# Yzmblog/SurfD

Measured on AMD Instinct MI355X. Metric: shapes/sec end-to-end (1000-step uncond, 512^3 UDF) at 1/2/4/8 GPU, higher is better.
Workload: dtype f32 (every matrix product of decoder and denoiser as three split-fp16 products on the fp16 MFMA pipe with fp32 accumulation — fp32-class error, same golden tolerances as the exact-fp32 kernels; samplers, attention, embedding MLP and grid bookkeeping in exact fp32)

## Files before the change

surfd_amd/csrc/conv_f16x2.hip:

```cpp
#include "common.h"
#include "unet_api.h"
#include "unet_plan.h"
#include <string.h>
#include <stdlib.h>
#include <algorithm>
#include <type_traits>

namespace surfd {

typedef _Float16 f16x8 __attribute__((ext_vector_type(8)));
typedef f16x8 __attribute__((address_space(1))) gf16x8;
typedef _Float16 f16x2 __attribute__((ext_vector_type(2)));
typedef float f32x2 __attribute__((ext_vector_type(2)));

struct Seg2 {
    const float *x;
    long bstride;
    const float *gamma, *beta;
    int C, Lin, log2Lin;
    int taps, stride, ups, gn, act;
    int blk, blkp, nblk;
    int k16_off;
    int gs;
    int log2P, gsm;
};

struct Conv2Args {
    Seg2 seg[2];
    int nseg;
    const _Float16 *whf;
    int KS16;
#if defined(SURFD_C2_PROBE) || defined(SURFD_C2_DBG_POISON)
    unsigned long long *probe;
#define C2_LDS_BYTES plane
#else
    const float *sc;
#endif
    float inv_sc;
    const float *bias;
    const float *emb;
    long emb_bstride;
    const float *res;
    long res_bstride;
    int res_cstride, res_lstride, has_res, has_emb;
    float *out;
    long out_bstride;
    int Cout, Lout, log2Lout, B;
    int bchunk, Lsl, cs;
    int plane;
    int off_ex, off_red;
    int ntiles, nby, KS;
    int nrt;
    int nhalf;
    unsigned magic_nby, magic_ks, magic_g;
    float *part;
    int part_stride;
    int *counters;
    const int *step_ptr;
    long emb_step_stride;
// ... 263 lines not shown
        "s_mov_b32 s66, %0\n\ts_mov_b32 s67, %0\n\ts_mov_b32 s68, %0\n\ts_mov_b32 s69, %0\n\ts_mov_b32 s70, %0\n\ts_mov_b32 s71, %0\n\t"
        "s_mov_b32 s72, %0\n\ts_mov_b32 s73, %0\n\ts_mov_b32 s74, %0\n\ts_mov_b32 s75, %0\n\ts_mov_b32 s76, %0\n\ts_mov_b32 s77, %0\n\t"
        "s_mov_b32 s78, %0\n\ts_mov_b32 s79, %0\n\ts_mov_b32 s80, %0\n\ts_mov_b32 s81, %0\n\ts_mov_b32 s82, %0\n\ts_mov_b32 s83, %0\n\t"
        "s_mov_b32 s84, %0\n\ts_mov_b32 s85, %0\n\ts_mov_b32 s86, %0\n\ts_mov_b32 s87, %0\n\ts_mov_b32 s88, %0\n\ts_mov_b32 s89, %0\n\t"
        "s_mov_b32 s90, %0\n\ts_mov_b32 s91, %0\n\ts_mov_b32 s92, %0\n\ts_mov_b32 s93, %0\n\ts_mov_b32 s94, %0\n\ts_mov_b32 s95, %0\n\t"
        "s_mov_b32 s96, %0\n\ts_mov_b32 s97, %0\n\ts_mov_b32 s98, %0\n\ts_mov_b32 s99, %0\n\t"
        "s_nop 0"
        :: "s"(pat)
        :
          "v1","v2","v3","v4","v5","v6","v7","v8","v9","v10","v11","v12","v13","v14","v15","v16","v17","v18","v19","v20","v21","v22","v23","v24",
          "v25","v26","v27","v28","v29","v30","v31","v32","v33","v34","v35","v36","v37","v38","v39","v40","v41","v42","v43","v44","v45","v46","v47","v48",
          "v49","v50","v51","v52","v53","v54","v55","v56","v57","v58","v59","v60","v61","v62","v63","v64","v65","v66","v67","v68","v69","v70","v71","v72",
          "v73","v74","v75","v76","v77","v78","v79","v80","v81","v82","v83","v84","v85","v86","v87","v88","v89","v90","v91","v92","v93","v94","v95","v96",
          "v97","v98","v99","v100","v101","v102","v103","v104","v105","v106","v107","v108","v109","v110","v111","v112","v113","v114","v115","v116","v117","v118","v119","v120",
          "v121","v122","v123","v124","v125","v126","v127","v128","v129","v130","v131","v132","v133","v134","v135","v136","v137","v138","v139","v140","v141","v142","v143","v144",
          "v145","v146","v147","v148","v149","v150","v151","v152","v153","v154","v155","v156","v157","v158","v159",
          "s4","s5","s6","s7","s8","s9","s10","s11","s12","s13","s14","s15","s16","s17","s18","s19","s20","s21","s22","s23","s24","s25","s26","s27",
          "s28","s29","s30","s31","s34","s35","s36","s37","s38","s39","s40","s41","s42","s43","s44","s45","s46","s47","s48","s49","s50","s51","s52","s53",
          "s54","s55","s56","s57","s58","s59","s60","s61","s62","s63","s64","s65","s66","s67","s68","s69","s70","s71","s72","s73","s74","s75","s76","s77",
          "s78","s79","s80","s81","s82","s83","s84","s85","s86","s87","s88","s89","s90","s91","s92","s93","s94","s95","s96","s97","s98","s99");
}
#endif

template <int VEC, bool PREF, bool WT = false, bool LEAN = false, bool LF = false, bool NT2 = false>
__global__ __launch_bounds__(256, LEAN ? SURFD_C2_LEAN_WAVES : (VEC == 16 ? (WT ? 2 : 1) : 2)) void conv2_kernel(Conv2Args A) {
    static_assert(!LEAN || (WT && VEC == 8 && !PREF), "lean form: wide decomposition, rows of <= 32 positions, no operand prefetch");
    static_assert(!NT2 || (LEAN && !LF), "two column tiles per wave: lean form only");
    constexpr int NCT = NT2 ? 2 : 1;
    [[maybe_unused]] constexpr int EXS = NT2 ? 128 : 256;
    constexpr bool SLIM = LEAN || (WT && VEC == 16);
    constexpr bool ONE_ACC = NT2 || (LEAN && SURFD_C2_LEAN_U == 3);
    constexpr int C2_U = (LEAN && !NT2) ? SURFD_C2_LEAN_U : SLIM ? 2 : 4;
    constexpr int C2_D = (VEC == 8 && SURFD_C2_EPI_LATE && !LEAN && !LF) ? (WT ? SURFD_C2_DEEP_D : SURFD_C2_LAT_D) : 2;
    [[maybe_unused]] constexpr bool ALIAS = SLIM;
    extern __shared__ __attribute__((aligned(16))) char lds_raw[];
    _Float16 *slab = reinterpret_cast<_Float16 *>(lds_raw);
#if !SURFD_C2_GNW
    float *ex_mean = reinterpret_cast<float *>(lds_raw + (ALIAS ? 0 : A.off_ex));
    float *ex_m2 = ex_mean + VEC * 256;
    float *gstat = ex_m2 + VEC * 256;
#endif
    float *red = reinterpret_cast<float *>(lds_raw + A.off_red);

#if defined(SURFD_C2_DBG_POISON) && SURFD_C2_DBG_POISON
    c2_poison_registers<!LEAN>();
    for (int e = threadIdx.x; e < A.C2_LDS_BYTES / 4; e += 256) reinterpret_cast<unsigned *>(lds_raw)[e] = SURFD_C2_DBG_POISON == 2 ? 0x7fc00000u : 0u;
    lds_bar();
#endif
    c2_kernarg_prefetch<(int)sizeof(Conv2Args)>();
    const int tid = threadIdx.x, lane = tid & 63;
    const int wave = __builtin_amdgcn_readfirstlane(tid >> 6);
#ifdef SURFD_C2_STAMPS
    long long stamp_[12];
#pragma unroll
    for (int i = 0; i < 12; ++i) stamp_[i] = 0;
#define C2_STAMP(i) do { stamp_[i] = (long long)__builtin_amdgcn_s_memrealtime(); } while (0)
#define C2_STAMP_FIRST(i) do { if (ch == kz) C2_STAMP(i); } while (0)
#else
#define C2_STAMP(i) do { } while (0)
#define C2_STAMP_FIRST(i) do { } while (0)
#endif
    C2_STAMP(0);
#ifdef SURFD_C2_STAMPS
    const long long cyc0_ = (long long)__builtin_readcyclecounter();
#endif
    int tile, by, kz, rg;
    bool tile_ok = true;
    {
        const int bid = blockIdx.x;
        const int G = A.nrt * A.KS;
        int g;
        if (G < 8) {
            by = G == 1 ? bid : (int)__umulhi((unsigned)bid, A.magic_g);
            g = bid - by * G;
        } else {
            const int xcd = bid & 7, idx = bid >> 3;
            const int j = A.nby == 1 ? idx : (int)__umulhi((unsigned)idx, A.magic_nby);
            by = idx - j * A.nby;
            g = xcd + 8 * j;
            if (g >= G) return;
        }
        rg = A.KS == 1 ? g : (int)__umulhi((unsigned)g, A.magic_ks);
        kz = g - rg * A.KS;
        tile = rg;
        if constexpr (WT) {
            tile = rg * 4 + wave;
            tile_ok = tile < A.ntiles;
            tile = min(tile, A.ntiles - 1);
        }
    }
    const bool halves = WT && A.nhalf == 2;
// ... 14 lines not shown
        const int lp = A.seg[s].log2P, gsm = A.seg[s].gsm;
        const int pos = lane & ((1 << lp) - 1);
        const int c = ((wc << (6 - lp)) + (lane >> lp)) * gsm + pos;
        ok = pos < gsm && c < A.seg[s].blk;
        return c;
#else
        ok = zthr < A.seg[s].blk;
        return zthr;
#endif
    };
    int colb[NCT], coll[NCT];
#pragma unroll
    for (int t = 0; t < NCT; ++t) {
        int m = (NT2 ? t : ct) * 32 + (lane & 31);
        if (m >= M) m = 0;
        m += m_off;
        colb[t] = m >> A.log2Lout;
        coll[t] = m & (A.Lout - 1);
    }
    const int nblk0 = A.seg[0].nblk;
    const int nch = nblk0 + (A.nseg > 1 ? A.seg[1].nblk : 0);
    constexpr int PLANE = NT2 ? C2_PLANE_NT2 : LEAN ? C2_PLANE_LEAN : (VEC == 16 ? 18432 : 15360);
    const int cs = A.cs;
    const float inv_sc = A.inv_sc;

    f32x16 acc_hh[NCT], acc_sm[1];
#pragma unroll
    for (int t = 0; t < NCT; ++t)
#pragma unroll
        for (int r = 0; r < 16; ++r) acc_hh[t][r] = 0.f;
    if constexpr (!ONE_ACC)
#pragma unroll
        for (int r = 0; r < 16; ++r) acc_sm[0][r] = 0.f;

    struct WS { const _Float16 *base; int it_beg, it_end, ngroups, nk; };
    auto make_ws = [&](int ch) -> WS {
        const int s = ch >= nblk0 ? 1 : 0;
        const int bi = ch - (s ? nblk0 : 0);
        const int nk = A.seg[s].blkp >> 4;
        const int iters = A.seg[s].taps * nk;
        const int per = (iters + KP - 1) >> log2kp;
        WS w;
        w.nk = nk;
        w.it_beg = min(kpart * per, iters);
        w.it_end = min(iters, w.it_beg + per);
        w.ngroups = (per + C2_U - 1) / C2_U;
// ... 17 lines not shown

    auto issue_operand = [&](int ch, f32x4 (&v)[VEC], float &ga, float &be) {
        const int s = ch >= nblk0 ? 1 : 0;
        const int bi = ch - (s ? nblk0 : 0);
        const int lv = A.seg[s].log2Lin - 2;
        const int Lin = A.seg[s].Lin;
        bool cok_;
        const int cg = min(bi * A.seg[s].blk + min(chan_of(s, cok_), A.seg[s].blk - 1), A.seg[s].C - 1);
        const float *src = A.seg[s].x + (long)cg * Lin;
        const long bstride = A.seg[s].bstride;
        const int rowbase = rhalf * ((VEC * 4) >> A.seg[s].log2Lin);
#pragma unroll
        for (int j = 0; j < VEC; ++j) {
            const int i = min(rowbase + (j >> lv), nb - 1), jj = j & ((1 << lv) - 1);
            v[j] = *reinterpret_cast<const f32x4 *>(src + (b0 + i) * bstride + 4 * jj);
        }
        ga = A.seg[s].gamma[cg]; be = A.seg[s].beta[cg];
    };

    int ch = kz;
    WS cur = make_ws(ch);
    f32x4 v[VEC];
    float ga, be;
    issue_operand(ch, v, ga, be);
#pragma unroll
    for (int d = 0; d < C2_D; ++d) load_group(ring[d], cur.base, cur.it_beg + d * C2_U, cur.it_end - 1);
    unsigned pf_sink[C2_PFN_N];
    if constexpr (SURFD_C2_PFN_FORMS || LEAN) c2_prefetch_next(A, tid, pf_sink);
    else {
#pragma unroll
        for (int k = 0; k < C2_PFN_N; ++k) pf_sink[k] = 0u;
    }

    f32x4 pre_b[4], pre_e[NCT][4];
    float pre_r[NCT][16];
    const float *embp = A.emb;
    if (A.step_ptr) embp += (long)(*reinterpret_cast<const __attribute__((address_space(4))) int *>((unsigned long)A.step_ptr)) * A.emb_step_stride;
    LoopFuse lfv;
    int lfk = 0;
    float lfrow[5] = {0.f, 0.f, 0.f, 0.f, 0.f};
    if constexpr (LF) {
        lfv = *A.lf;
        lfk = *lfv.step;
#pragma unroll
        for (int q = 0; q < 5; ++q) lfrow[q] = lfv.tab[(long)lfk * 8 + q];
    }
    auto request_epilogue = [&]() {
        const int cmax4 = ((A.Cout + 3) & ~3) - 4;
#pragma unroll
        for (int t = 0; t < NCT; ++t) {
            const int m = min((NT2 ? t : ct) * 32 + (lane & 31), M - 1) + m_off;
// ... 26 lines not shown
#pragma unroll
        for (int qq = 0; qq < 2; ++qq) {
            const int q = kpart * QN + min(qq, QN - 1);
            const int cob = min(tile * 32 + 8 * q + 4 * (lane >> 5), cmax4);
            dpre_b[qq] = *reinterpret_cast<const f32x4 *>(A.bias + cob);
            dpre_e[qq] = *reinterpret_cast<const f32x4 *>(embp + b * A.emb_bstride + cob);
#pragma unroll
            for (int k = 0; k < 4; ++k) {
                const int co = min(cob + k, A.Cout - 1);
                dpre_r[qq][k] = A.res[b * A.res_bstride + (long)co * A.res_cstride + l * A.res_lstride];
            }
        }
    };
    constexpr bool EPI_LATE = SLIM || SURFD_C2_EPI_LATE;
    if constexpr (!EPI_LATE && !DIST) request_epilogue();
    bool saturated = false;
    C2_STAMP(1);
#ifdef SURFD_C2_PROBE
    unsigned long long probe_w = 0ull;
#endif

    while (true) {
        {
            const int s = ch >= nblk0 ? 1 : 0;
            const int bi = ch - (s ? nblk0 : 0);
            const int lv = A.seg[s].log2Lin - 2, vpr = 1 << lv;
            const int Lin = A.seg[s].Lin;
            const int blk = A.seg[s].blk, blkp = A.seg[s].blkp;
            bool cok;
            const int c = chan_of(s, cok);
            const int rowbase = rhalf * ((VEC * 4) >> A.seg[s].log2Lin);
            const int pad = A.seg[s].taps == 3 ? 1 : 0;
            const int ups = A.seg[s].ups, act = A.seg[s].act;
#ifdef SURFD_C2_PROBE
            {
                unsigned long long h = 0ull;
#pragma unroll
                for (int j = 0; j < VEC; ++j)
#pragma unroll
                    for (int k = 0; k < 4; ++k) h += (unsigned long long)__float_as_uint(v[j][k]) * (unsigned long long)(2 * ((ch * 256 + tid) * 64 + j * 4 + k) + 1);
                h += (unsigned long long)__float_as_uint(ga) * 7ull + (unsigned long long)__float_as_uint(be) * 11ull;
                C2_PROBE_ADD(0, h);
            }
#endif
            if (A.seg[s].gn) {
                const int gs = A.seg[s].gs;
// ... 187 lines not shown
                                const f32x2 hf = __builtin_convertvector(h, f32x2);
                                const f16x2 lo = __builtin_convertvector(w - hf, f16x2);
                                _Float16 *d0 = row + (k * RS) * cs, *d1 = d0 + RS * cs;
                                d0[0] = h[0]; d0[PLANE] = lo[0];
                                d1[0] = h[1]; d1[PLANE] = lo[1];
                                if constexpr (UPS) { d0[cs] = h[0]; d0[cs + PLANE] = lo[0]; d1[cs] = h[1]; d1[cs + PLANE] = lo[1]; }
                            }
                        }
                    }
                };
                if (ups) split_rows(std::true_type{}); else split_rows(std::false_type{});
                saturated |= amax > 65504.f;
            }
            if (zthr >= blk && zthr < blkp) {
                for (int i = 0; i < nb; ++i)
                    for (int p = 0; p < A.Lsl; ++p) { slab[(i * A.Lsl + p) * cs + zthr] = (_Float16)0.f; slab[(i * A.Lsl + p) * cs + zthr + PLANE] = (_Float16)0.f; }
            }
            if (cok)
                for (int i = 0; i < nb; ++i) {
                    _Float16 *row0 = slab + (i * A.Lsl) * cs + c;
                    for (int p = 0; p < pad; ++p) { row0[p * cs] = (_Float16)0.f; row0[p * cs + PLANE] = (_Float16)0.f; }
                    for (int p = pad + Lcov; p < A.Lsl; ++p) { row0[p * cs] = (_Float16)0.f; row0[p * cs + PLANE] = (_Float16)0.f; }
                }
            lds_bar();
            C2_STAMP_FIRST(4);
#ifdef SURFD_C2_PROBE
            {
                unsigned long long h = 0ull;
                const int n = nb * A.Lsl * blkp;
                for (int e = tid; e < n; e += 256) {
                    const int cch = e % blkp, rp = e / blkp;
                    const unsigned short hi = __builtin_bit_cast(unsigned short, slab[rp * cs + cch]), lo = __builtin_bit_cast(unsigned short, slab[rp * cs + cch + PLANE]);
                    h += ((unsigned long long)hi + 65537ull * lo) * (unsigned long long)(2 * (ch * 65536 + e) + 1);
                }
                C2_PROBE_ADD(3, h);
                lds_bar();
            }
#endif
        }
        const int chn = ch + A.KS;
        const bool has_next = chn < nch;
        const WS nxt = has_next ? make_ws(chn) : cur;
        f32x4 vn[PREF ? VEC : 1];
        float gan = 0.f, ben = 0.f;
        if constexpr (PREF) issue_operand(has_next ? chn : ch, vn, gan, ben);
        {
            const int s = ch >= nblk0 ? 1 : 0;
            int lbase[NCT];
#pragma unroll
            for (int t = 0; t < NCT; ++t) lbase[t] = (colb[t] * A.Lsl + coll[t] * A.seg[s].stride) * cs + 8 * (lane >> 5);
// ... 72 lines not shown
#pragma unroll
                for (int d = 0; d < C2_D; ++d) {
                    const int g = g0 + d;
                    compute(ring[d], g);
                    const int vg = g + C2_D;
                    const bool into_next = has_next && vg >= P;
                    const _Float16 *rb = into_next ? nxt.base : cur.base;
                    const int it0 = into_next ? nxt.it_beg + (vg - P) * C2_U : cur.it_beg + vg * C2_U;
                    const int itl = into_next ? nxt.it_end - 1 : cur.it_end - 1;
                    load_group(ring[d], rb, it0, itl);
                }
                g0 += C2_D;
            } while (g0 < P);
        }
        C2_STAMP_FIRST(5);
        if (!has_next) break;
        lds_bar();
        ch = chn;
        cur = nxt;
        if constexpr (PREF) {
#pragma unroll
            for (int j = 0; j < VEC; ++j) v[j] = vn[j];
            ga = gan; be = ben;
        } else {
            issue_operand(ch, v, ga, be);
        }
    }
    if constexpr (DIST) request_epilogue_dist();
    else if constexpr (EPI_LATE) request_epilogue();
    if (saturated) atomicAdd(A.sat, 1u);
    C2_STAMP(6);

    if constexpr (DIST) {
        lds_bar();
        {
            float *dst = red + (kpart * nct + ct) * 1024;
#pragma unroll
            for (int r = 0; r < 16; ++r) dst[r * 64 + lane] = ONE_ACC ? acc_hh[0][r] : acc_sm[0][r] + acc_hh[0][r];
        }
        lds_bar();
        f32x4 val[2];
#pragma unroll
        for (int qq = 0; qq < 2; ++qq) {
            const int q = kpart * QN + min(qq, QN - 1);
            const float *srcp = red + ct * 1024 + (4 * q) * 64 + lane;
            f32x4 t = {srcp[0], srcp[64], srcp[128], srcp[192]};
            for (int kp = 1; kp < KP; ++kp) {
// ... 199 lines not shown
            const int prev = __hip_atomic_fetch_add(lfv.done, 1, __ATOMIC_RELAXED, __HIP_MEMORY_SCOPE_AGENT);
            if (prev == A.nby * A.nrt - 1) {
                __hip_atomic_store(lfv.done, 0, __ATOMIC_RELAXED, __HIP_MEMORY_SCOPE_AGENT);
                __hip_atomic_store(lfv.step, lfk + 1, __ATOMIC_RELAXED, __HIP_MEMORY_SCOPE_AGENT);
            }
        }
    }
    {
        unsigned used = 0u;
#pragma unroll
        for (int k = 0; k < C2_PFN_N; ++k) used |= pf_sink[k];
        asm volatile("" :: "v"(used));
    }
#ifdef SURFD_C2_STAMPS
    C2_STAMP(9);
    asm volatile("s_waitcnt vmcnt(0)" ::: "memory");
    C2_STAMP(10);
    if (A.dbg && blockIdx.x == 0 && tid == 0) {
        for (int i = 0; i < 11; ++i) A.dbg[i] = stamp_[i];
        A.dbg[15] = (long long)__builtin_readcyclecounter() - cyc0_;
    }
#endif
}

__global__ void c2_hash_kernel(const float *p, long bstride, int B, int row, unsigned long long *out) {
    unsigned long long h = 0ull;
    const long n = (long)B * row;
    for (long e = blockIdx.x * (long)blockDim.x + threadIdx.x; e < n; e += (long)gridDim.x * blockDim.x) {
        const long b = e / row, r = e - b * row;
        h += (unsigned long long)__float_as_uint(p[b * bstride + r]) * (unsigned long long)(2 * e + 1);
    }
#pragma unroll
    for (int off = 32; off > 0; off >>= 1) h += __shfl_xor(h, off);
    if ((threadIdx.x & 63) == 0) atomicAdd(out, h);
}

__global__ void c2_absmax_kernel(const float *src, size_t n, unsigned *out) {
    unsigned m = 0u;
    for (size_t i = blockIdx.x * (size_t)blockDim.x + threadIdx.x; i < n; i += (size_t)gridDim.x * blockDim.x)
        m = max(m, __float_as_uint(src[i]) & 0x7fffffffu);
#pragma unroll
    for (int off = 32; off > 0; off >>= 1) m = max(m, (unsigned)__shfl_xor((int)m, off));
    if ((threadIdx.x & 63) == 0 && m) atomicMax(out, m);
}

__global__ void c2_scale_kernel(float *sc) {
// ... 303 lines not shown
    } else {
        if (base < ks_min_base && nch > 1) KS = std::min({nch, ks_max, std::max(1, ks_fill / base)});
        if ((size_t)KS * base * A.part_stride > u->part_floats || base > 8192) KS = 1;
    }
    A.KS = KS;
    static const int deep_below = env_int("SURFD_CONV2_DEEP_BELOW", 0);
    if (lean && !nt2 && deep_below > 0 && (long)A.nrt * KS * A.nby <= (long)deep_below * u->cu_budget) {
        lean = false;
        lds = (size_t)15360 * 2 * sizeof(_Float16);
        lds = (lds + 15) & ~(size_t)15;
        A.plane = 15360; A.off_ex = (int)lds; A.off_red = (int)lds;
#if SURFD_C2_GNW
        lds += (size_t)(4 * 1024 + 4) * sizeof(float);
#else
        lds += std::max(((size_t)2 * VEC * 256 + 2 * 8 * 32) * sizeof(float), (size_t)(3 * 1024 + 4) * sizeof(float));
#endif
        lds += (size_t)lds_extra;
        lds = (lds + 255) & ~(size_t)255;
        A.off_pf = (int)lds;
        lds += 256;
    }
    A.part = u->part; A.counters = u->counters;
    A.sat = u->sat;
    if (fuse_head) {
        if (io.ext_out_bs != (long)c.Cout * A.Lout) SURFD_FAIL(SURFD_ERR_ARG, "conv: fused posterior update needs a contiguous head output");
        A.lf = io.lf;
        if (io.lf_done) *io.lf_done = true;
    }
    A.dbg = nullptr;
    if (u->dbg && u->dbg_launch < 4096) {
        A.dbg = u->dbg + (size_t)(u->dbg_launch++) * 16;
        long long meta[4] = {c.Cout, c.seg[0].C + (c.nseg > 1 ? c.seg[1].C : 0), A.Lout * 100000LL + (long long)A.ntiles * A.nby * KS, KS * 100 + nch};
        HIP_TRY(hipMemcpyAsync(A.dbg + 11, meta, sizeof(meta), hipMemcpyHostToDevice, st));
    }
    A.magic_nby = (unsigned)((0x100000000ULL + A.nby - 1) / A.nby);
    A.magic_ks = (unsigned)((0x100000000ULL + KS - 1) / KS);
    const int G = A.nrt * KS;
    A.magic_g = (unsigned)((0x100000000ULL + G - 1) / G);
    if ((long)G * A.nby >= 65536) SURFD_FAIL(SURFD_ERR_UNSUPPORTED, "conv: %d x %d workgroups exceed the kernel's block decode", G, A.nby);
    dim3 grid((unsigned)(G < 8 ? G * A.nby : 8 * ceil_div(G, 8) * A.nby));
    static const int pref = env_int("SURFD_CONV2_PREF", 0);
    static const int wpref = env_int("SURFD_CONV2_WIDE_PREF", 0);
    {
        ConvPlan::LaunchRec &R = c.rec;
        R.gen = u->ws_gen; R.B = B; R.L = L; R.whf = A.whf; R.ntiles = A.ntiles; R.KS16 = A.KS16; R.tpg = wt ? 4 : 1; R.KS = KS; R.G = A.nrt * KS;
        R.nblk0 = A.seg[0].nblk; R.it0 = A.seg[0].taps * (A.seg[0].blkp >> 4);
// ... 11 lines not shown
            A.pf_w = reinterpret_cast<const char *>(R.whf);
            A.pf_ntiles = R.ntiles; A.pf_KS16 = R.KS16; A.pf_KS = R.KS; A.pf_G = R.G;
            A.pf_nblk0 = R.nblk0; A.pf_it0 = R.it0; A.pf_nch = R.nch; A.pf_it1 = std::max(R.it1, 1);
            auto lg = [](int v) { int l = 0; while ((1 << l) < v) ++l; return l; };
            A.pf_log2tpg = lg(R.tpg); A.pf_log2bps = lg(ceil_div(R.nch, R.KS)); A.pf_log2lpb = lg(16 * std::max(R.it0, R.it1));
            A.pf_magic_ks = (unsigned)((0x100000000ULL + R.KS - 1) / R.KS);
        }
    }
#if defined(SURFD_C2_PROBE) || defined(SURFD_C2_DBG_POISON)
    {
        static unsigned long long *const probe_base = [] { const char *e = getenv("SURFD_CONV2_PROBE_PTR"); return e ? reinterpret_cast<unsigned long long *>(strtoull(e, nullptr, 0)) : nullptr; }();
        A.probe = (probe_base && grid.x <= 4096 && c.id < 128) ? probe_base + (size_t)c.id * 4096 * 8 : nullptr;
        A.C2_LDS_BYTES = (int)lds;
    }
#endif
    auto launch = [&]() {
        if (A.lf) {
            if (wt && VEC == 16) hipLaunchKernelGGL((conv2_kernel<16, false, true, false, true>), grid, dim3(256), lds, st, A);
            else if (wt) hipLaunchKernelGGL((conv2_kernel<8, false, true, false, true>), grid, dim3(256), lds, st, A);
            else if (VEC == 16) hipLaunchKernelGGL((conv2_kernel<16, false, false, false, true>), grid, dim3(256), lds, st, A);
            else hipLaunchKernelGGL((conv2_kernel<8, false, false, false, true>), grid, dim3(256), lds, st, A);
        }
        else if (nt2) hipLaunchKernelGGL((conv2_kernel<8, false, true, true, false, true>), grid, dim3(256), lds, st, A);
        else if (lean) hipLaunchKernelGGL((conv2_kernel<8, false, true, true>), grid, dim3(256), lds, st, A);
        else if (wt && VEC == 16) hipLaunchKernelGGL((conv2_kernel<16, false, true>), grid, dim3(256), lds, st, A);
        else if (wt && wpref) hipLaunchKernelGGL((conv2_kernel<8, true, true>), grid, dim3(256), lds, st, A);
        else if (wt) hipLaunchKernelGGL((conv2_kernel<8, false, true>), grid, dim3(256), lds, st, A);
        else if (VEC == 16) hipLaunchKernelGGL((conv2_kernel<16, false>), grid, dim3(256), lds, st, A);
        else if (pref) hipLaunchKernelGGL((conv2_kernel<8, true>), grid, dim3(256), lds, st, A);
        else hipLaunchKernelGGL((conv2_kernel<8, false>), grid, dim3(256), lds, st, A);
    };
    launch();
    LAUNCH_CHECK();
    static const int hash_env = env_int("SURFD_CONV2_HASH", 0);
    if (hash_env && A.dbg) {
        HIP_TRY(hipMemsetAsync(A.dbg, 0, sizeof(long long), st));
        hipLaunchKernelGGL(c2_hash_kernel, dim3(64), dim3(256), 0, st, (const float *)A.out, (long)A.out_bstride, B, A.Cout * A.Lout,
                           reinterpret_cast<unsigned long long *>(A.dbg));
        LAUNCH_CHECK();
    }
    static const int twice = env_int("SURFD_CONV2_TWICE", 0);
    if (twice && !A.lf) {
        if (A.dbg && u->dbg_launch < 4096) {
            long long *prev = A.dbg;
            A.dbg = u->dbg + (size_t)(u->dbg_launch++) * 16;
            HIP_TRY(hipMemcpyAsync(A.dbg + 11, prev + 11, 4 * sizeof(long long), hipMemcpyDeviceToDevice, st));
        }
        launch();
    }
    LAUNCH_CHECK();
    return SURFD_OK;
}

#define C2_STR_(x) #x
// ... 28 lines not shown
#error "SURFD_C2_GNPAD=0: the in-wave GroupNorm reductions without wait states are NOT bit-stable run to run (profiles/r05_loop_experiments.md section 3, profiles/r06_conv2_instability.md); -DSURFD_ALLOW_UNSAFE_VARIANTS builds it anyway"
#endif
#if SURFD_C2_LAT_D != 2
#error "SURFD_C2_LAT_D != 2 is not a validated configuration of the latency form (profiles/r05_loop_experiments.md section 1); -DSURFD_ALLOW_UNSAFE_VARIANTS builds it anyway"
#endif
#if SURFD_C2_BPIPE == 2
#error "SURFD_C2_BPIPE=2 is the control of an experiment (not bit-stable with SURFD_C2_GNW, profiles/r06_conv2_instability.md); -DSURFD_ALLOW_UNSAFE_VARIANTS builds it anyway"
#endif
#if C2_CFG_ABLATE != 0 || C2_CFG_POISON != 0 || C2_CFG_PROBE != 0
#error "developer aids of conv_f16x2.hip (SURFD_C2_ABLATE / _DBG_POISON / _PROBE) change results or timing; -DSURFD_ALLOW_UNSAFE_VARIANTS builds them anyway"
#endif
#endif
const char *conv2_build_config() {
    return "C2_GNW=" C2_STR(SURFD_C2_GNW) " C2_BPIPE=" C2_STR(SURFD_C2_BPIPE) " C2_GNPAD=" C2_STR(SURFD_C2_GNPAD) " C2_PFN=" C2_STR(SURFD_C2_PFN) " C2_PFN_FORMS=" C2_STR(SURFD_C2_PFN_FORMS)
           " C2_PFN_N=" C2_STR(SURFD_C2_PFN_N) " C2_KAPF=" C2_STR(SURFD_C2_KAPF)
           " C2_FAST_RCP=" C2_STR(SURFD_C2_FAST_RCP) " C2_EPI_LATE=" C2_STR(SURFD_C2_EPI_LATE) " C2_LAT_D=" C2_STR(SURFD_C2_LAT_D) " C2_DEEP_D=" C2_STR(SURFD_C2_DEEP_D)
           " C2_ZB=" C2_STR(SURFD_C2_ZB) " C2_DIST=" C2_STR(SURFD_C2_DIST) " C2_LEAN_WAVES=" C2_STR(SURFD_C2_LEAN_WAVES) " C2_LEAN_U=" C2_STR(SURFD_C2_LEAN_U) " C2_PLANE_LEAN=" C2_STR(SURFD_C2_PLANE_LEAN)
           " C2_ABLATE=" C2_STR(C2_CFG_ABLATE) " C2_DBG_POISON=" C2_STR(C2_CFG_POISON) " C2_PROBE=" C2_STR(C2_CFG_PROBE) " C2_STAMPS=" C2_STR(C2_CFG_STAMPS);
}
int conv2_build_unsafe() { return C2_UNSAFE_COUNT; }

int conv2_set_attributes() {
    const int max_lds = 160 * 1024;
    HIP_TRY(hipFuncSetAttribute(reinterpret_cast<const void *>(&conv2_kernel<8, true>), hipFuncAttributeMaxDynamicSharedMemorySize, max_lds));
    HIP_TRY(hipFuncSetAttribute(reinterpret_cast<const void *>(&conv2_kernel<8, false>), hipFuncAttributeMaxDynamicSharedMemorySize, max_lds));
    HIP_TRY(hipFuncSetAttribute(reinterpret_cast<const void *>(&conv2_kernel<16, false>), hipFuncAttributeMaxDynamicSharedMemorySize, max_lds));
    HIP_TRY(hipFuncSetAttribute(reinterpret_cast<const void *>(&conv2_kernel<8, false, true>), hipFuncAttributeMaxDynamicSharedMemorySize, max_lds));
    HIP_TRY(hipFuncSetAttribute(reinterpret_cast<const void *>(&conv2_kernel<8, true, true>), hipFuncAttributeMaxDynamicSharedMemorySize, max_lds));
    HIP_TRY(hipFuncSetAttribute(reinterpret_cast<const void *>(&conv2_kernel<8, false, true, true>), hipFuncAttributeMaxDynamicSharedMemorySize, max_lds));
    HIP_TRY(hipFuncSetAttribute(reinterpret_cast<const void *>(&conv2_kernel<8, false, true, true, false, true>), hipFuncAttributeMaxDynamicSharedMemorySize, max_lds));
    HIP_TRY(hipFuncSetAttribute(reinterpret_cast<const void *>(&conv2_kernel<8, false, true, false, true>), hipFuncAttributeMaxDynamicSharedMemorySize, max_lds));
    HIP_TRY(hipFuncSetAttribute(reinterpret_cast<const void *>(&conv2_kernel<16, false, true>), hipFuncAttributeMaxDynamicSharedMemorySize, max_lds));
    HIP_TRY(hipFuncSetAttribute(reinterpret_cast<const void *>(&conv2_kernel<16, false, true, false, true>), hipFuncAttributeMaxDynamicSharedMemorySize, max_lds));
    HIP_TRY(hipFuncSetAttribute(reinterpret_cast<const void *>(&conv2_kernel<16, false, false, false, true>), hipFuncAttributeMaxDynamicSharedMemorySize, max_lds));
    HIP_TRY(hipFuncSetAttribute(reinterpret_cast<const void *>(&conv2_kernel<8, false, false, false, true>), hipFuncAttributeMaxDynamicSharedMemorySize, max_lds));
    return SURFD_OK;
}

}
```

surfd_amd/csrc/unet.hip:

```cpp
#include "common.h"
#include "unet_api.h"
#include "unet_plan.h"
#include <string.h>
#include <algorithm>
#include <stdlib.h>

namespace surfd {

struct SegArgs {
    const float *x;
    long bstride;
    int C, Cp;
    int Lin;
    int taps, stride, ups;
    int gn, act;
    int bmod;
    const float *gamma, *beta;
    int kg_off;
    int cc;
    const float *add;
    long add_step_stride;
};

struct ConvArgs {
// ... 627 lines not shown
    u->ops.push_back(a);
    Op b; b.kind = 0;
    ConvPlan &c2 = b.conv;
    c2.Cout = cout; c2.ds_out = ds;
    c2.seg[0].src = View{scratch1, 0}; c2.seg[0].C = cout; c2.seg[0].taps = 3; c2.seg[0].gn = 1; c2.seg[0].act = 1; c2.seg[0].ds = ds;
    c2.seg[0].wkey = p + ".out_layers.3.weight"; c2.seg[0].gnkey = p + ".out_layers.0";
    c2.bias_keys = {p + ".out_layers.3.bias"};
    if (cin != cout) {
        c2.nseg = 2;
        c2.seg[1].src = src; c2.seg[1].C = cin; c2.seg[1].taps = 1; c2.seg[1].ds = ds;
        c2.seg[1].wkey = p + ".skip_connection.weight";
        c2.bias_keys.push_back(p + ".skip_connection.bias");
    } else {
        c2.nseg = 1;
        c2.res = src;
    }
    c2.dst = dst;
    u->ops.push_back(b);
}

void emit_attn(surfd_unet *u, const std::string &p, View src, int c, int ds, int qkv_buf, int att_buf, View dst) {
    Op a; a.kind = 0;
    ConvPlan &q = a.conv;
    q.Cout = 3 * c; q.ds_out = ds;
    q.seg[0].src = src; q.seg[0].C = c; q.seg[0].taps = 1; q.seg[0].gn = 1; q.seg[0].act = 0; q.seg[0].ds = ds;
    q.seg[0].wkey = p + ".qkv.weight"; q.seg[0].gnkey = p + ".norm";
    q.bias_keys = {p + ".qkv.bias"};
    q.dst = View{qkv_buf, 0};
    u->ops.push_back(a);
    Op m; m.kind = 1;
    m.attn.qkv = View{qkv_buf, 0}; m.attn.out = View{att_buf, 0}; m.attn.C = c; m.attn.ds = ds;
    u->ops.push_back(m);
    Op b; b.kind = 0;
    ConvPlan &pr = b.conv;
    pr.Cout = c; pr.ds_out = ds;
    pr.seg[0].src = View{att_buf, 0}; pr.seg[0].C = c; pr.seg[0].taps = 1; pr.seg[0].ds = ds;
    pr.seg[0].wkey = p + ".proj_out.weight";
    pr.bias_keys = {p + ".proj_out.bias"};
    pr.res = src; pr.dst = dst;
    u->ops.push_back(b);
}

void emit_plain_conv(surfd_unet *u, const std::string &wprefix, View src, int cin, int cout, int ds_src, int ds_out,
                     int stride, int ups, View dst) {
    Op a; a.kind = 0;
    ConvPlan &c = a.conv;
    c.Cout = cout; c.ds_out = ds_out;
// ... 218 lines not shown

int surfd_unet_create(const surfd_unet_cfg *cfg, surfd_unet **out) {
    if (!cfg || !out) SURFD_FAIL(SURFD_ERR_ARG, "surfd_unet_create: null argument");
    if (cfg->n_mult < 1 || cfg->n_mult > 8 || cfg->n_attn < 0 || cfg->n_attn > 8 || cfg->num_heads < 1 ||
        cfg->model_channels % 32 || cfg->model_channels % cfg->num_heads || cfg->num_res_blocks < 1)
        SURFD_FAIL(SURFD_ERR_UNSUPPORTED, "surfd_unet_create: unsupported configuration");
    auto *u = new surfd_unet();
    u->cfg = *cfg;
    int rc = build_plan(u);
    if (rc) { delete u; return rc; }
    *out = u;
    return SURFD_OK;
}

void surfd_unet_destroy(surfd_unet *u) {
    if (!u) return;
    if (u->wpack) (void)hipFree(u->wpack);
    if (u->vecs) (void)hipFree(u->vecs);
    if (u->label_table) (void)hipFree(u->label_table);
    for (float *p : u->buf_ptr) if (p) (void)hipFree(p);
    for (float *p : {u->temb, u->h1, u->emb, u->emb_table, u->emb_ctx}) if (p) (void)hipFree(p);
    if (u->t_dev) (void)hipFree(u->t_dev);
    if (u->part) (void)hipFree(u->part);
    if (u->counters) (void)hipFree(u->counters);
    for (void *p : {(void *)u->whf, (void *)u->whf2, (void *)u->wsc, (void *)u->sat}) if (p) (void)hipFree(p);
    if (u->loop.exec) (void)hipGraphExecDestroy(u->loop.exec);
    if (u->loop.graph) (void)hipGraphDestroy(u->loop.graph);
    if (u->loop.cap_stream) (void)hipStreamDestroy(u->loop.cap_stream);
    if (u->loop.poll_stream) (void)hipStreamDestroy(u->loop.poll_stream);
    for (void *p : {(void *)u->loop.step_ctr, (void *)u->loop.x, (void *)u->loop.x0, u->loop.params, (void *)u->loop.tab}) if (p) (void)hipFree(p);
    delete u;
}

int surfd_unet_num_params(const surfd_unet *u) { return u ? (int)u->params.size() : 0; }

int surfd_unet_param_info(const surfd_unet *u, int i, const char **key, int64_t shape[4], int *ndim) {
    if (!u || i < 0 || i >= (int)u->params.size()) SURFD_FAIL(SURFD_ERR_ARG, "surfd_unet_param_info: bad index %d", i);
    *key = u->params[i].key.c_str();
    *ndim = (int)u->params[i].shape.size();
    for (int j = 0; j < *ndim; ++j) shape[j] = u->params[i].shape[j];
    return SURFD_OK;
}

int surfd_unet_set_param(surfd_unet *u, const char *key, const void *dev_ptr, const int64_t *shape, int ndim, surfd_stream s) {
    if (!u || !key || !dev_ptr) SURFD_FAIL(SURFD_ERR_ARG, "surfd_unet_set_param: null argument");
    std::string k(key);
// ... 530 lines not shown
```

surfd_amd/csrc/unet_plan.h:

```cpp
#pragma once
#include "common.h"
#include "unet_api.h"

namespace surfd {

struct ParamInfo {
    std::string key;
    std::vector<int64_t> shape;
    bool is_set = false;
};

struct View { int buf = -1; int choff = 0; };

struct BufInfo { int C; int ds; };

struct SegPlan {
    View src;
    int C = 0, taps = 1, stride = 1, ups = 0, gn = 0, act = 0;
    std::string wkey;
    std::string gnkey;
    int ds = 1;
};

struct ConvPlan {
    SegPlan seg[2];
    int nseg = 1;
    int Cout = 0;
    int ds_out = 1;
    std::vector<std::string> bias_keys;
    int emb_off = -1;
    View res, dst;
    size_t w_off = 0; int KGtot = 0; int kg_off[2] = {0, 0}; size_t bias_off = 0; int gn_off[2] = {-1, -1};
    int f16_ok = 0;
    int blk[2] = {0, 0}, blkp[2] = {0, 0}, nblk[2] = {0, 0}, k16_off[2] = {0, 0};
    int KS16 = 0;
    size_t whf_off = 0;
    int sc_idx = -1;
    int id = -1;
    int f16_ok2 = 0;
    int blk2[2] = {0, 0}, blkp2[2] = {0, 0}, nblk2[2] = {0, 0}, k16_off2[2] = {0, 0};
    int KS16_2 = 0;
    size_t whf2_off = 0;
    struct LaunchRec {
        long gen = -1; int B = 0, L = 0;
        const _Float16 *whf = nullptr;
        int ntiles = 0, KS16 = 0, tpg = 1, KS = 1, G = 1, nblk0 = 0, it0 = 0, nch = 0, it1 = 0;
    };
    mutable LaunchRec rec;
};

struct AttnPlan { View qkv, out; int C = 0, ds = 1; };

struct Op { int kind; ConvPlan conv; AttnPlan attn; };

}

struct surfd_unet {
    using ParamInfo = surfd::ParamInfo; using BufInfo = surfd::BufInfo; using Op = surfd::Op; using ConvPlan = surfd::ConvPlan;
    surfd_unet_cfg cfg;
    int ted = 0;
    std::vector<ParamInfo> params;
    std::map<std::string, int> pindex;
    std::vector<BufInfo> bufs;
    std::vector<Op> ops;
    ConvPlan lin1, lin2, lin3;
    int emb_total = 0;
    std::vector<std::pair<std::string, int>> emb_layers;
    bool allocated = false, finalized = false;
    int device = -1;
    float *wpack = nullptr; size_t wpack_floats = 0;
    float *vecs = nullptr; size_t vec_floats = 0;
    std::map<std::string, size_t> vec_off;
    float *label_table = nullptr;
    std::vector<float *> buf_ptr; int ws_B = 0, ws_L = 0;
    float *temb = nullptr, *h1 = nullptr, *emb = nullptr, *emb_table = nullptr; int emb_rows_cap = 0; int emb_rows = 0, emb_B = 0;
    int emb_shared = 0;
    int emb_ingraph = 0;
    float *emb_ctx = nullptr; int emb_ctx_cap = 0;
    int64_t *t_dev = nullptr; int t_cap = 0;
    float *part = nullptr; size_t part_floats = 0;
    long long *dbg = nullptr; int dbg_launch = 0;
    surfd::LoopState loop;
    int *counters = nullptr;
    _Float16 *whf = nullptr; size_t whf_halfs = 0;
    _Float16 *whf2 = nullptr; size_t whf2_halfs = 0;
    float *wsc = nullptr; int n_sc = 0;
    std::vector<float> wsc_host;
    unsigned *sat = nullptr;
    int wide_batch = 0;
    int cu_budget = 256;
    int precision = 1;
    int dbg_only = -1;
    const surfd::ConvPlan *pf_next = nullptr;
    long ws_gen = 1;
};


namespace surfd {
int conv2_plan_layout(surfd_unet *u);
int conv2_finalize(surfd_unet *u, hipStream_t st);
int conv2_set_attributes();
struct ConvLaunchIO {
    const float *ext_in; long ext_in_bs;
// ... 9 lines not shown
```

Baseline: 4.876.

## Pre-stage attention QKV operand into global fp16 image via separate stager kernel

For the attention QKV projection conv (1x1, groupnorm, no activation), a separate stager launch first builds the split-fp16 hi/lo operand slabs for every batch-chunk and channel block into a global buffer. The main lean kernel then copies these prebuilt images into LDS instead of recomputing the normalization and conversion in each tile block. This removes work that every column/K-split block repeated. In exchange it adds an extra kernel launch and a global scratch round-trip, and the scratch buffer is lazily allocated, which bumps the workspace generation.

Result: no change. 4.871 (-0.1%).

```diff
diff --git a/surfd_amd/csrc/conv_f16x2.hip b/surfd_amd/csrc/conv_f16x2.hip
--- a/surfd_amd/csrc/conv_f16x2.hip
+++ b/surfd_amd/csrc/conv_f16x2.hip
@@ -34,7 +34,10 @@
     unsigned long long *probe;
 #define C2_LDS_BYTES plane
 #else
-    const float *sc;
+    union {
+        const float *sc;
+        _Float16 *pre;
+    };
 #endif
     float inv_sc;
     const float *bias;
@@ -344,10 +347,22 @@
 }
 #endif
 
-template <int VEC, bool PREF, bool WT = false, bool LEAN = false, bool LF = false, bool NT2 = false>
-__global__ __launch_bounds__(256, LEAN ? SURFD_C2_LEAN_WAVES : (VEC == 16 ? (WT ? 2 : 1) : 2)) void conv2_kernel(Conv2Args A) {
+#ifndef SURFD_C2_PRESTAGE
+#define SURFD_C2_PRESTAGE 1
+#endif
+#if defined(SURFD_C2_PROBE) || defined(SURFD_C2_DBG_POISON) || (defined(SURFD_C2_GNW) && !SURFD_C2_GNW)
+#undef SURFD_C2_PRESTAGE
+#define SURFD_C2_PRESTAGE 0
+#endif
+
+constexpr int C2_VEC8_PRE = 8 + 256 * 1, C2_VEC8_STAGER = 8 + 256 * 2;
+template <int VECM, bool PREF, bool WT = false, bool LEAN = false, bool LF = false, bool NT2 = false>
+__global__ __launch_bounds__(256, LEAN ? SURFD_C2_LEAN_WAVES : ((VECM & 255) == 16 ? (WT ? 2 : 1) : 2)) void conv2_kernel(Conv2Args A) {
+    constexpr int VEC = VECM & 255, MODE = VECM >> 8;
     static_assert(!LEAN || (WT && VEC == 8 && !PREF), "lean form: wide decomposition, rows of <= 32 positions, no operand prefetch");
     static_assert(!NT2 || (LEAN && !LF), "two column tiles per wave: lean form only");
+    static_assert(MODE == 0 || (LEAN && !NT2 && !LF), "pre-staged operand: lean one-tile wide form only");
+    constexpr bool PRE = MODE == 1, STAGER = MODE == 2;
     constexpr int NCT = NT2 ? 2 : 1;
     [[maybe_unused]] constexpr int EXS = NT2 ? 128 : 256;
     constexpr bool SLIM = LEAN || (WT && VEC == 16);
@@ -388,7 +403,9 @@
 #endif
     int tile, by, kz, rg;
     bool tile_ok = true;
-    {
+    if constexpr (STAGER) {
+        by = blockIdx.x; kz = blockIdx.y; rg = 0; tile = 0;
+    } else {
         const int bid = blockIdx.x;
         const int G = A.nrt * A.KS;
         int g;
@@ -449,6 +466,10 @@
     const int nch = nblk0 + (A.nseg > 1 ? A.seg[1].nblk : 0);
     constexpr int PLANE = NT2 ? C2_PLANE_NT2 : LEAN ? C2_PLANE_LEAN : (VEC == 16 ? 18432 : 15360);
     const int cs = A.cs;
+#if SURFD_C2_PRESTAGE
+    [[maybe_unused]] auto image_of = [&](int ch) -> _Float16 * { return A.pre + ((size_t)by * nch + ch) * (size_t)(2 * PLANE); };
+    if constexpr (STAGER) slab = image_of(kz);
+#endif
     const float inv_sc = A.inv_sc;
 
     f32x16 acc_hh[NCT], acc_sm[1];
@@ -512,11 +533,12 @@
     WS cur = make_ws(ch);
     f32x4 v[VEC];
     float ga, be;
-    issue_operand(ch, v, ga, be);
+    if constexpr (!PRE) issue_operand(ch, v, ga, be);
+    if constexpr (!STAGER)
 #pragma unroll
     for (int d = 0; d < C2_D; ++d) load_group(ring[d], cur.base, cur.it_beg + d * C2_U, cur.it_end - 1);
     unsigned pf_sink[C2_PFN_N];
-    if constexpr (SURFD_C2_PFN_FORMS || LEAN) c2_prefetch_next(A, tid, pf_sink);
+    if constexpr (!STAGER && (SURFD_C2_PFN_FORMS || LEAN)) c2_prefetch_next(A, tid, pf_sink);
     else {
 #pragma unroll
         for (int k = 0; k < C2_PFN_N; ++k) pf_sink[k] = 0u;
@@ -589,6 +611,25 @@
 
     while (true) {
         {
+#if SURFD_C2_PRESTAGE
+            if constexpr (PRE) {
+                constexpr int NCP = (PLANE / 8 + 255) / 256;
+                const int n8 = (nb * A.Lsl * cs) >> 3;
+                const gf16x8 *src = (const gf16x8 *)image_of(ch);
+                f16x8 th[NCP], tl[NCP];
+#pragma unroll
+                for (int k = 0; k < NCP; ++k) {
+                    const int e = min(tid + 256 * k, n8 - 1);
+                    th[k] = src[e];
+                    tl[k] = src[PLANE / 8 + e];
+                }
+                f16x8 *dst = reinterpret_cast<f16x8 *>(slab);
+#pragma unroll
+                for (int k = 0; k < NCP; ++k)
+                    if (tid + 256 * k < n8) { dst[tid + 256 * k] = th[k]; dst[PLANE / 8 + tid + 256 * k] = tl[k]; }
+            } else
+#endif
+            {
             const int s = ch >= nblk0 ? 1 : 0;
             const int bi = ch - (s ? nblk0 : 0);
             const int lv = A.seg[s].log2Lin - 2, vpr = 1 << lv;
@@ -822,10 +863,16 @@
                     for (int p = 0; p < pad; ++p) { row0[p * cs] = (_Float16)0.f; row0[p * cs + PLANE] = (_Float16)0.f; }
                     for (int p = pad + Lcov; p < A.Lsl; ++p) { row0[p * cs] = (_Float16)0.f; row0[p * cs + PLANE] = (_Float16)0.f; }
                 }
+            }
+            if constexpr (STAGER) {
+                if (saturated) atomicAdd(A.sat, 1u);
+                return;
+            }
             lds_bar();
             C2_STAMP_FIRST(4);
 #ifdef SURFD_C2_PROBE
             {
+                const int blkp = A.seg[ch >= nblk0 ? 1 : 0].blkp;
                 unsigned long long h = 0ull;
                 const int n = nb * A.Lsl * blkp;
                 for (int e = tid; e < n; e += 256) {
@@ -944,7 +991,7 @@
 #pragma unroll
             for (int j = 0; j < VEC; ++j) v[j] = vn[j];
             ga = gan; be = ben;
-        } else {
+        } else if constexpr (!PRE) {
             issue_operand(ch, v, ga, be);
         }
     }
@@ -1190,6 +1237,7 @@
     }
 #endif
 }
+
 
 __global__ void c2_hash_kernel(const float *p, long bstride, int B, int row, unsigned long long *out) {
     unsigned long long h = 0ull;
@@ -1539,6 +1587,21 @@
     }
     A.part = u->part; A.counters = u->counters;
     A.sat = u->sat;
+    bool prestage = false;
+#if SURFD_C2_PRESTAGE
+    prestage = c.attn_qkv && lean && !nt2 && !fuse_head && c.nseg == 1 && c.seg[0].taps == 1 && c.seg[0].gn && !c.seg[0].act && !c.seg[0].ups;
+    if (prestage) {
+        const size_t need = (size_t)ceil_div(std::max(B, u->wide_batch), nb) * nch * 2 * C2_PLANE_LEAN;
+        if (need > u->pre_halfs) {
+            if (u->pre) { HIP_TRY(hipFree(u->pre)); u->pre = nullptr; u->pre_halfs = 0; }
+            HIP_TRY(hipMalloc((void **)&u->pre, need * sizeof(_Float16)));
+            HIP_TRY(hipMemset(u->pre, 0, need * sizeof(_Float16)));
+            u->pre_halfs = need;
+            u->ws_gen++;
+        }
+        A.pre = u->pre;
+    }
+#endif
     if (fuse_head) {
         if (io.ext_out_bs != (long)c.Cout * A.Lout) SURFD_FAIL(SURFD_ERR_ARG, "conv: fused posterior update needs a contiguous head output");
         A.lf = io.lf;
@@ -1596,6 +1659,9 @@
             else hipLaunchKernelGGL((conv2_kernel<8, false, false, false, true>), grid, dim3(256), lds, st, A);
         }
         else if (nt2) hipLaunchKernelGGL((conv2_kernel<8, false, true, true, false, true>), grid, dim3(256), lds, st, A);
+#if SURFD_C2_PRESTAGE
+        else if (prestage) hipLaunchKernelGGL((conv2_kernel<C2_VEC8_PRE, false, true, true>), grid, dim3(256), lds, st, A);
+#endif
         else if (lean) hipLaunchKernelGGL((conv2_kernel<8, false, true, true>), grid, dim3(256), lds, st, A);
         else if (wt && VEC == 16) hipLaunchKernelGGL((conv2_kernel<16, false, true>), grid, dim3(256), lds, st, A);
         else if (wt && wpref) hipLaunchKernelGGL((conv2_kernel<8, true, true>), grid, dim3(256), lds, st, A);
@@ -1604,6 +1670,12 @@
         else if (pref) hipLaunchKernelGGL((conv2_kernel<8, true>), grid, dim3(256), lds, st, A);
         else hipLaunchKernelGGL((conv2_kernel<8, false>), grid, dim3(256), lds, st, A);
     };
+#if SURFD_C2_PRESTAGE
+    if (prestage) {
+        hipLaunchKernelGGL((conv2_kernel<C2_VEC8_STAGER, false, true, true>), dim3((unsigned)A.nby, (unsigned)nch), dim3(256), 0, st, A);
+        LAUNCH_CHECK();
+    }
+#endif
     launch();
     LAUNCH_CHECK();
     static const int hash_env = env_int("SURFD_CONV2_HASH", 0);
@@ -1678,6 +1750,9 @@
 
 int conv2_set_attributes() {
     const int max_lds = 160 * 1024;
+#if SURFD_C2_PRESTAGE
+    HIP_TRY(hipFuncSetAttribute(reinterpret_cast<const void *>(&conv2_kernel<C2_VEC8_PRE, false, true, true>), hipFuncAttributeMaxDynamicSharedMemorySize, max_lds));
+#endif
     HIP_TRY(hipFuncSetAttribute(reinterpret_cast<const void *>(&conv2_kernel<8, true>), hipFuncAttributeMaxDynamicSharedMemorySize, max_lds));
     HIP_TRY(hipFuncSetAttribute(reinterpret_cast<const void *>(&conv2_kernel<8, false>), hipFuncAttributeMaxDynamicSharedMemorySize, max_lds));
     HIP_TRY(hipFuncSetAttribute(reinterpret_cast<const void *>(&conv2_kernel<16, false>), hipFuncAttributeMaxDynamicSharedMemorySize, max_lds));
@@ -1690,6 +1765,9 @@
     HIP_TRY(hipFuncSetAttribute(reinterpret_cast<const void *>(&conv2_kernel<16, false, true, false, true>), hipFuncAttributeMaxDynamicSharedMemorySize, max_lds));
     HIP_TRY(hipFuncSetAttribute(reinterpret_cast<const void *>(&conv2_kernel<16, false, false, false, true>), hipFuncAttributeMaxDynamicSharedMemorySize, max_lds));
     HIP_TRY(hipFuncSetAttribute(reinterpret_cast<const void *>(&conv2_kernel<8, false, false, false, true>), hipFuncAttributeMaxDynamicSharedMemorySize, max_lds));
+#if SURFD_C2_PRESTAGE
+    HIP_TRY(hipFuncSetAttribute(reinterpret_cast<const void *>(&conv2_kernel<C2_VEC8_PRE, false, true, true>), hipFuncAttributeMaxDynamicSharedMemorySize, max_lds));
+#endif
     return SURFD_OK;
 }
 
diff --git a/surfd_amd/csrc/unet.hip b/surfd_amd/csrc/unet.hip
--- a/surfd_amd/csrc/unet.hip
+++ b/surfd_amd/csrc/unet.hip
@@ -673,7 +673,7 @@
 void emit_attn(surfd_unet *u, const std::string &p, View src, int c, int ds, int qkv_buf, int att_buf, View dst) {
     Op a; a.kind = 0;
     ConvPlan &q = a.conv;
-    q.Cout = 3 * c; q.ds_out = ds;
+    q.Cout = 3 * c; q.ds_out = ds; q.attn_qkv = 1;
     q.seg[0].src = src; q.seg[0].C = c; q.seg[0].taps = 1; q.seg[0].gn = 1; q.seg[0].act = 0; q.seg[0].ds = ds;
     q.seg[0].wkey = p + ".qkv.weight"; q.seg[0].gnkey = p + ".norm";
     q.bias_keys = {p + ".qkv.bias"};
@@ -938,6 +938,7 @@
     for (float *p : {u->temb, u->h1, u->emb, u->emb_table, u->emb_ctx}) if (p) (void)hipFree(p);
     if (u->t_dev) (void)hipFree(u->t_dev);
     if (u->part) (void)hipFree(u->part);
+    if (u->pre) (void)hipFree(u->pre);
     if (u->counters) (void)hipFree(u->counters);
     for (void *p : {(void *)u->whf, (void *)u->whf2, (void *)u->wsc, (void *)u->sat}) if (p) (void)hipFree(p);
     if (u->loop.exec) (void)hipGraphExecDestroy(u->loop.exec);
diff --git a/surfd_amd/csrc/unet_plan.h b/surfd_amd/csrc/unet_plan.h
--- a/surfd_amd/csrc/unet_plan.h
+++ b/surfd_amd/csrc/unet_plan.h
@@ -37,6 +37,7 @@
     size_t whf_off = 0;
     int sc_idx = -1;
     int id = -1;
+    int attn_qkv = 0;
     int f16_ok2 = 0;
     int blk2[2] = {0, 0}, blkp2[2] = {0, 0}, nblk2[2] = {0, 0}, k16_off2[2] = {0, 0};
     int KS16_2 = 0;
@@ -79,6 +80,7 @@
     float *emb_ctx = nullptr; int emb_ctx_cap = 0;
     int64_t *t_dev = nullptr; int t_cap = 0;
     float *part = nullptr; size_t part_floats = 0;
+    _Float16 *pre = nullptr; size_t pre_halfs = 0;
     long long *dbg = nullptr; int dbg_launch = 0;
     surfd::LoopState loop;
     int *counters = nullptr;
```
